# zitongbai/bipedal_control

Measured on AMD Instinct MI355X. Metric: MPC solves/s (H1, horizon=100), higher is better.
Workload: dtype f64; 1 GPU; Unitree H1 trot (template tiled from t = 0), horizon=100 intervals (dt 0.015), batch=256 per GPU perturbed initial states, cold start, 1 SQP iteration (BASELINE.json configs[1]); solver=sqp, global_batch=256, problems_on_rank0=256, shooting_nodes=108, nx=22, nu=22

## Files before the change

bipedal_control_amd/csrc/k_node.hip:

```cpp
#include <hip/hip_runtime.h>
#include <hip/hip_ext.h>

#include <stdexcept>

#include "kernel_launchers.h"
#include "launch.h"
#include "kernels/rollout.h"

namespace bpmpc {

template <int NJ>
__global__ __launch_bounds__(kWave) void k_prepare(Launch L) {
  constexpr int NX = 12 + NJ, NU = 12 + NJ;
  const int s = blockIdx.x, b = s / L.N, k = s % L.N;
  const int g = L.buf.p_grid[b];
  const int n = L.buf.g_nodes[g];
  if (k >= n) { if (threadIdx.x == 0) L.buf.n_info[s] = 0; return; }
  const size_t gs = (size_t)g * L.N + k;
  if (threadIdx.x == 0) L.buf.n_info[s] = 8 | ((L.buf.g_mode[gs] & 3) << 1) | (L.buf.g_kind[gs] == 1 ? 1 : 0);
  if (threadIdx.x < kNodeAux) {
    const int t = threadIdx.x;
    L.buf.n_aux[(size_t)s * kNodeAux + t] = t == 0 ? L.buf.g_dt[gs] : t < 5 ? L.buf.g_zref[gs * 4 + t - 1] : t < 9 ? L.buf.g_zdref[gs * 4 + t - 5] : 0.0;
  }
  prepare_node<NJ>(*L.model, L.buf.g_kind[gs], L.buf.g_mode[gs], L.buf.g_start[gs], L.cold != 0, k == n - 1, L.buf.p_tgt_n[b],
// ... 198 lines not shown
  constexpr int NX = 12 + NJ, NU = 12 + NJ, LPN = C::LPN, NPW = C::NPW;
  __shared__ LinFastNodeLds<NJ, false, CHAIN> lds[kTrialWaves * NPW];
  __shared__ LinFastShared<NJ, false> shared;
  const int sub = threadIdx.x / LPN, g = threadIdx.x % LPN;
  const int widx = blockIdx.x * (kTrialWaves * NPW) + sub;
  {
    const int total = L.batch * L.klen, w0 = blockIdx.x * (kTrialWaves * NPW), w1 = (w0 + kTrialWaves * NPW < total ? w0 + kTrialWaves * NPW : total) - 1;
    bool any = false;
    for (int pb = w0 / L.klen; pb <= w1 / L.klen; ++pb) any = any || L.buf.done[pb] == 0;
    if (!any) return;
  }
  bool valid = widx < L.batch * L.klen;
  const int b = valid ? widx / L.klen : 0, k = valid ? L.k0 + widx % L.klen : 0;
  const double* dx = L.buf.dx + ((size_t)b * (L.N + 1) + k) * NX;
  {
    const int fin = L.buf.done[b];
    const double alpha = L.buf.alpha[b];
    const int info = L.buf.n_info[(size_t)b * L.N + k];
    const size_t s0 = (size_t)b * L.N + k;
    const double* xk = L.buf.x + ((size_t)b * (L.N + 1) + k) * NX;
    const TrialPre pre = trial_preload<C>(xk, xk + NX, L.buf.u + s0 * NU, L.buf.xref + s0 * NX, dx, dx + NX, L.buf.du + s0 * NU, g, L.buf.n_aux + s0 * kNodeAux);
    load_shared_model<kTrialWaves * kWave>(*L.model, shared, threadIdx.x);
    NodeInputs in;
    in.kind = info & 1; in.mode = (info >> 1) & 3; in.dt = 0.0;
    in.x = xk; in.xnext = xk + NX; in.u = L.buf.u + s0 * NU; in.xref = L.buf.xref + s0 * NX; in.zref = nullptr; in.zdref = nullptr;
    __syncthreads();
    valid = valid && fin == 0 && info != 0;
    const size_t s = valid ? s0 : 0;
    trial_fast<NJ, C>(*L.model, shared, lds[sub], valid, in, alpha, dx, L.buf.du + s * NU, dx + NX, L.buf.trial_perf + s * 3, g, nullptr, &pre);
  }
}

template <int NJ, bool CHAIN>
__global__ __launch_bounds__(kTrialWaves * kWave) void k_constraint_values(Launch L, double* eqv) {
  using C = LinFastCfg<NJ, true, CHAIN>;
  constexpr int NX = 12 + NJ, NU = 12 + NJ, LPN = C::LPN, NPW = C::NPW;
  __shared__ LinFastNodeLds<NJ, false, CHAIN> lds[kTrialWaves * NPW];
  __shared__ LinFastShared<NJ, false> shared;
  load_shared_model<kTrialWaves * kWave>(*L.model, shared, threadIdx.x);
  __syncthreads();
  const int sub = threadIdx.x / LPN, g = threadIdx.x % LPN;
  const int widx = blockIdx.x * (kTrialWaves * NPW) + sub;
  bool valid = widx < L.batch * L.klen;
  const int b = valid ? widx / L.klen : 0, k = valid ? L.k0 + widx % L.klen : 0;
  const int grid = L.buf.p_grid[b];
  valid = valid && k < L.buf.g_nodes[grid] && L.buf.g_kind[(size_t)grid * L.N + k] == 0;
  const size_t s = valid ? (size_t)b * L.N + k : 0;
  const NodeInputs in = node_inputs<NJ>(L, b, k);
  const double* dx = L.buf.dx + ((size_t)b * (L.N + 1) + k) * NX;
  double perf[3];
  trial_fast<NJ, C, true>(*L.model, shared, lds[sub], valid, in, 0.0, dx, L.buf.du + s * NU, dx + NX, perf, g, eqv + s * kMaxEqRows);
}

template <int NJ, bool CHAIN>
__global__ __launch_bounds__(kWave) void k_rollout(const DeviceModel* model, RolloutArgs a) {
  __shared__ RolloutLds<NJ, CHAIN> w;
  load_shared_model<kWave>(*model, w.shared, threadIdx.x);
  __syncthreads();
  rollout_policy<NJ, CHAIN>(*model, w, a);
}

constexpr int kDecideThreads = 256;
template <int NJ>
__global__ __launch_bounds__(kDecideThreads) void k_ls_decide(Launch L, int look_first) {
  __shared__ double partial[3 * kDecideThreads + 5];
  linesearch_decide<NJ, kDecideThreads>(partial, problem_ls<NJ>(L, blockIdx.x), L.ls, look_first != 0);
// ... 75 lines not shown
      if (ev_start && ev_stop) hipExtLaunchKernelGGL(kernel, grid, block, 0, st, ev_start, ev_stop, 0, L);
      else hipLaunchKernelGGL(kernel, grid, block, 0, st, L);
    };
    if (L.ilqr) {
      if (!L.serial_legs) throw std::runtime_error("linearize_fast: the ILQR lineariser is instantiated for serial-leg robots only");
      if (materialise) launch(k_linearize_fast<NJ, true, true, true>);
      else launch(k_linearize_fast<NJ, false, true, true>);
    } else if (L.serial_legs) {
      if (materialise) launch(k_linearize_fast<NJ, true, true>);
      else launch(k_linearize_fast<NJ, false, true>);
    } else {
      if (materialise) launch(k_linearize_fast<NJ, true, false>);
      else launch(k_linearize_fast<NJ, false, false>);
    }
  });
}
void warm_shift(int nj, int slots, hipStream_t st, const Launch& L, const int* restarted) {
  KL_NJ(nj, hipLaunchKernelGGL(k_warm_shift<NJ>, dim3(slots), dim3(kWave), 0, st, L, restarted));
}
void ls_begin(int nj, int batch, hipStream_t st, const Launch& L) { KL_NJ(nj, hipLaunchKernelGGL(k_ls_begin<NJ>, dim3(batch), dim3(kWave), 0, st, L)); }
void trial_reference(int nj, int slots, hipStream_t st, const Launch& L) { KL_NJ(nj, hipLaunchKernelGGL(k_trial<NJ>, dim3(slots), dim3(kWave), 0, st, L)); }
int trial_fast_workgroups(int nj, int nodes) {
  const int per_wg = kTrialWaves * (nj == 10 ? LinFastCfg<10, true>::NPW : LinFastCfg<12, true>::NPW);
  return (nodes + per_wg - 1) / per_wg;
}
void trial_fast(int nj, int nodes, hipStream_t st, const Launch& L) {
  const int grid = trial_fast_workgroups(nj, nodes);
  KL_NJ(nj, {
    if (L.serial_legs) hipLaunchKernelGGL((k_trial_fast<NJ, true>), dim3(grid), dim3(kTrialWaves * kWave), 0, st, L);
    else hipLaunchKernelGGL((k_trial_fast<NJ, false>), dim3(grid), dim3(kTrialWaves * kWave), 0, st, L);
  });
}
void ls_decide(int nj, int batch, hipStream_t st, const Launch& L, bool look_first) { KL_NJ(nj, hipLaunchKernelGGL(k_ls_decide<NJ>, dim3(batch), dim3(kDecideThreads), 0, st, L, look_first ? 1 : 0)); }
void ls_tail(int nj, int batch, hipStream_t st, const Launch& L, int first_round, int max_trials, bool pending) {
  KL_NJ(nj, {
    if (L.serial_legs) hipLaunchKernelGGL((k_ls_tail<NJ, true>), dim3(batch), dim3(kTailThreads), 0, st, L, first_round, max_trials, pending ? 1 : 0);
    else hipLaunchKernelGGL((k_ls_tail<NJ, false>), dim3(batch), dim3(kTailThreads), 0, st, L, first_round, max_trials, pending ? 1 : 0);
  });
}
void constraint_values(int nj, int nodes, hipStream_t st, const Launch& L, double* eqv) {
  const int grid = trial_fast_workgroups(nj, nodes);
  KL_NJ(nj, {
    if (L.serial_legs) hipLaunchKernelGGL((k_constraint_values<NJ, true>), dim3(grid), dim3(kTrialWaves * kWave), 0, st, L, eqv);
    else hipLaunchKernelGGL((k_constraint_values<NJ, false>), dim3(grid), dim3(kTrialWaves * kWave), 0, st, L, eqv);
  });
}
void rollout(int nj, bool serial_legs, int batch, hipStream_t st, const DeviceModel* model, const RolloutArgs& a) {
  KL_NJ(nj, {
    constexpr bool kChainFits = LinFastCfg<NJ, false, true>::LPN == 16;
    const dim3 grid((batch + LinFastCfg<NJ>::NPW - 1) / LinFastCfg<NJ>::NPW);
    if constexpr (kChainFits) {
      if (serial_legs) { hipLaunchKernelGGL((k_rollout<NJ, true>), grid, dim3(kWave), 0, st, model, a); return; }
    }
    hipLaunchKernelGGL((k_rollout<NJ, false>), grid, dim3(kWave), 0, st, model, a);
  });
}
void copy_pairs(int grid, hipStream_t st, const double* a_src, double* a_dst, size_t na, const double* b_src, double* b_dst, size_t nb,
                int* iterations, int* active, int batch) {
  hipLaunchKernelGGL(k_copy_pairs, dim3(grid > 0 ? grid : 1), dim3(256), 0, st, a_src, a_dst, na, b_src, b_dst, nb, iterations, active, batch);
}

}
}
```

bipedal_control_amd/csrc/kernel_launchers.h:

```cpp
#pragma once
#include <hip/hip_runtime.h>

#include <cstddef>
#include <stdexcept>

namespace bpmpc {

#define KL_NJ(nj, ...)                                                          \
  do {                                                                          \
    if ((nj) == 10) { constexpr int NJ = 10; __VA_ARGS__; }                     \
    else if ((nj) == 12) { constexpr int NJ = 12; __VA_ARGS__; }                \
    else throw std::runtime_error("unsupported joint count");                   \
  } while (0)

struct Launch;
struct DeviceModel;
struct RolloutArgs;
struct DdpBuffers;
struct TickArgs;
struct RestartArgs;

namespace kl {

void prepare(int nj, int slots, hipStream_t st, const Launch& L);
void linearize_reference(int nj, int slots, hipStream_t st, const Launch& L);
void linearize_fast(int nj, bool materialise, int nodes, hipStream_t st, const Launch& L, hipEvent_t ev_start = nullptr, hipEvent_t ev_stop = nullptr);
void warm_shift(int nj, int slots, hipStream_t st, const Launch& L, const int* restarted = nullptr);
void ls_begin(int nj, int batch, hipStream_t st, const Launch& L);
void trial_reference(int nj, int slots, hipStream_t st, const Launch& L);
int trial_fast_workgroups(int nj, int nodes);
void trial_fast(int nj, int nodes, hipStream_t st, const Launch& L);
void ls_decide(int nj, int batch, hipStream_t st, const Launch& L, bool look_first = false);
void ls_tail(int nj, int batch, hipStream_t st, const Launch& L, int first_round, int max_trials, bool pending);
void constraint_values(int nj, int nodes, hipStream_t st, const Launch& L, double* eqv);
void rollout(int nj, bool serial_legs, int batch, hipStream_t st, const DeviceModel* model, const RolloutArgs& a);
void copy_pairs(int grid, hipStream_t st, const double* a_src, double* a_dst, size_t na, const double* b_src, double* b_dst, size_t nb,
                int* iterations, int* active, int batch);

void project_reference(int nj, int slots, hipStream_t st, const Launch& L);
void project_lu_s(int nj, int max_vel_rows, bool packed, int nodes, hipStream_t st, const Launch& L);
void project_fast(int nj, bool packed, bool joint_rows, int nodes, hipStream_t st, const Launch& L);

void riccati_reference(int nj, int batch, hipStream_t st, const Launch& L);
void riccati_fast(int nj, bool joint_rows, int batch, hipStream_t st, const Launch& L);
void riccati_fast8(int nj, bool joint_rows, int batch, hipStream_t st, const Launch& L);

void riccati_wave(int nj, bool two_per_simd, bool joint_rows, int batch, hipStream_t st, const Launch& L);
void riccati_rollout(int nj, int batch, hipStream_t st, const Launch& L);

void ddp_policy(int nj, int batch, hipStream_t st, const Launch& L, const DdpBuffers& d);
void ddp_cost(int nj, int batch, bool fast, hipStream_t st, const Launch& L, const DdpBuffers& d);
void ddp_select(int nj, int batch, hipStream_t st, const Launch& L, const DdpBuffers& d, double armijo);
void ddp_nominal(int nj, int batch, hipStream_t st, const Launch& L, const DdpBuffers& d);
void ddp_finish(int nj, int batch, hipStream_t st, const Launch& L, const DdpBuffers& d);
void ddp_keep_times(int batch, int N, hipStream_t st, const DdpBuffers& d, double* tp_time, int* tp_kind, int* tp_nodes, int* tp_grid);

void tick_observe_policy(int nj, int batch, hipStream_t st, const DeviceModel* model, const TickArgs& a);
void tick_commands(int nj, int batch, hipStream_t st, const double* x_opt, const double* u_opt, const double* sol, double* cmd);
void restart_observe(int nj, int batch, hipStream_t st, const DeviceModel* model, const RestartArgs& a);

}
}
```

bipedal_control_amd/csrc/kernels/linesearch.h:

```cpp
#pragma once
#include "node_lq.h"

namespace bpmpc {

constexpr int kMaxTargetPoints = 8;
constexpr int kStatsStride = 16;

struct LineSearchSettings {
  double g_max, g_min, alpha_decay, alpha_min, gamma_c, armijo_factor, delta_tol, cost_tol;
  int max_iterations;
};

template <int NJ>
BP_DEVICE void prepare_node(const DeviceModel& md, int kind, int mode, double t_start, bool cold, bool last, int n_pts, const double* tgt_t,
                            const double* tgt_x, const double* x0, double* xref, double* x, double* u, double* x_terminal) {
  constexpr int NX = 12 + NJ, NU = 12 + NJ;
  BP_LANES(tid, kWave) {
    if (tid < NX) {
      double val;
      if (n_pts == 1 || t_start <= tgt_t[0]) {
        val = tgt_x[tid];
      } else if (t_start >= tgt_t[n_pts - 1]) {
        val = tgt_x[(n_pts - 1) * NX + tid];
      } else {
// ... 170 lines not shown
#if defined(BPMPC_HOST_EMULATION)
        p.remaining[0] -= 1;
#else
        atomicSub(p.remaining, 1);
#endif
      } else {
        p.alpha[0] = next_alpha;
      }
    }
  }
  BP_SYNC();
  const bool accepted = partial[3 * NL] != 0.0;
  if (accepted) {
#if !defined(BPMPC_HOST_EMULATION)
#pragma unroll
    for (int j = 0; j < UPD; ++j) {
      const int idx = (int)threadIdx.x + j * NL;
      if (idx < nxe) p.x[idx] = xv[j] + alpha * dxv[j];
      if (idx < nue) p.u[idx] = uv[j] + alpha * duv[j];
    }
    int t0 = (int)threadIdx.x;
    if constexpr (!PRE) asm volatile("" : "+v"(t0));
    for (int idx = t0 + UPD * NL; idx < nxe; idx += NL) p.x[idx] += alpha * p.dx[idx];
    for (int idx = t0 + UPD * NL; idx < nue; idx += NL) p.u[idx] += alpha * p.du[idx];
#else
    BP_LANES(tid, NL) {
      for (int idx = tid; idx < (p.n_nodes + 1) * NX; idx += NL) p.x[idx] += alpha * p.dx[idx];
      for (int idx = tid; idx < p.n_nodes * NU; idx += NL) p.u[idx] += alpha * p.du[idx];
    }
#endif
  }
}

}
```

bipedal_control_amd/csrc/launch.h:

```cpp
#pragma once
#include <hip/hip_runtime.h>

#include <cstddef>

#include "device_model.h"
#include "kernels/linesearch.h"
#include "kernels/node_lq.h"
#include "kernels/project_node.h"
#include "kernels/riccati_fast.h"
#include "kernels/linearize_fast.h"

namespace bpmpc {

struct Buffers {
  int *g_kind, *g_mode, *g_nodes;
  double *g_dt, *g_start, *g_zref, *g_zdref;
  int* p_grid;
  double *p_x0, *p_tgt_t, *p_tgt_x;
  int* p_tgt_n;
  double *x, *u, *x_init, *u_init, *xref;
  double *A, *B, *b, *Q, *R, *P, *q, *r, *c, *C, *D, *e, *perf;
  int* nc;
  double *Px, *Pu, *Pe, *At, *Bt, *bt, *Qt, *Rt, *Pt, *qt, *rt;
  double *Wt, *Qp, *Mt;
  double* Vt;
  int* nut;
  int* n_info;
  double* n_aux;
  double* lin_park;
  double* lin_dump;
  double* qrd;
  double *Kt, *kt, *dx, *du, *K, *summary, *dx0;
  double *Acl, *bcl, *kff, *mvec, *mscal, *rprof;
  double *x_prev, *u_prev, *K_prev, *tp_time;
  int *tp_kind, *tp_nodes, *tp_grid;
  double *roll_t, *roll_x0, *roll_x, *roll_u;
  int *roll_steps, *roll_status;
  double *g_time, *rg_t0, *rg_start, *p_t0, *p_cmd, *lib_d;
  int *rg_gait, *rg_status, *rg_rows, *lib_i;
  double* ric_carry;
  double* zero_page;
  double *trial_perf, *base, *alpha, *stats;
  int *done, *active, *iterations, *remaining;
};

struct DdpBuffers {
  int cap;
  int nv;
  double alpha_v[kMaxDdpSteps];
  double* lff;
  double *rec_t, *rec_x, *rec_u, *cost;
  int* rec_n;
  double *end_x, *end_u;
  int *roll_steps, *roll_status;
  double *sol_t, *sol_x, *sol_u;
  int* sol_n;
  double *merit0, *merit, *alpha, *update_is;
  int *accepted, *failed, *n_points;
};

constexpr int kLinMaxEvents = 8;
struct Launch {
  const DeviceModel* model;
  Buffers buf;
  int batch, N;
  int k0, klen;
  int cold;
  int feedback;
  int serial_legs;
  LineSearchSettings ls;
  double reg_prim;
  int lin_ev_n, lin_inter;
  int lin_ev[kLinMaxEvents];
  int ilqr;
  double ilqr_shift;
};
// ... 41 lines not shown
  const size_t s0 = (size_t)b * L.N;
  p.n_nodes = L.buf.g_nodes[L.buf.p_grid[b]];
  p.node_perf = L.buf.perf + s0 * 3;
  p.trial_perf = L.buf.trial_perf + s0 * 3;
  p.x0 = L.buf.p_x0 + (size_t)b * NX;
  p.x = L.buf.x + (size_t)b * (L.N + 1) * NX;
  p.u = L.buf.u + s0 * NU;
  p.dx = L.buf.dx + (size_t)b * (L.N + 1) * NX;
  p.du = L.buf.du + s0 * NU;
  p.summary = L.buf.summary + (size_t)b * 4;
  p.base = L.buf.base + (size_t)b * 3;
  p.alpha = L.buf.alpha + b;
  p.done = L.buf.done + b;
  p.active = L.buf.active + b;
  p.iterations = L.buf.iterations + b;
  p.stats = L.buf.stats + (size_t)b * kStatsStride;
  p.remaining = L.buf.remaining;
  return p;
}

template <int NJ>
__device__ __forceinline__ bool riccati_fast_io(const Launch& L, RiccatiFastIO& io, double* lds_scratch ) {
  constexpr int NX = 12 + NJ, NU = 12 + NJ;
  const int b = blockIdx.x;
  const int tid_ = threadIdx.x;
  io.with_ls = L.k0 == 0;
  if (io.with_ls) io.ls = problem_ls<NJ>(L, b);
  if (!L.buf.active[b]) {
    if (io.with_ls && tid_ < kWave) linesearch_begin_wave<NJ>(lds_scratch, io.ls, tid_);
    return false;
  }
  const size_t s0 = (size_t)b * L.N;
  double* dx0 = L.buf.dx0 + (size_t)b * NX;
  if (tid_ < NX) dx0[tid_] = L.buf.p_x0[(size_t)b * NX + tid_] - L.buf.x[(size_t)b * (L.N + 1) * NX + tid_];
  __syncthreads();
  io.base.N = L.buf.g_nodes[L.buf.p_grid[b]];
  io.base.nut = L.buf.nut + s0;
  io.base.At = L.buf.At + s0 * NX * NX; io.base.Bt = L.buf.Bt + s0 * NX * NU; io.base.bt = L.buf.bt + s0 * NX;
  io.base.Qt = L.buf.Qt + s0 * NX * NX; io.base.Rt = L.buf.Rt + s0 * NU * NU; io.base.Pt = L.buf.Pt + s0 * NU * NX;
  io.base.qt = L.buf.qt + s0 * NX; io.base.rt = L.buf.rt + s0 * NU;
  io.Wt = L.buf.Wt + s0 * PackedLq<NJ>::W_SIZE; io.Qp = L.buf.Qp + s0 * PackedLq<NJ>::Q_SIZE; io.Mt = L.buf.Mt + s0 * PackedLq<NJ>::M_SIZE;
  io.base.Px = L.buf.Px + s0 * NU * NX; io.base.Pu = L.buf.Pu + s0 * NU * NU; io.base.Pe = L.buf.Pe + s0 * NU;
  io.Vt = L.buf.Vt + s0 * NJ * PackedLq<NJ>::WP;
  io.mode = L.buf.g_mode + (size_t)L.buf.p_grid[b] * L.N;
  io.zero_one = L.buf.zero_page;
  io.lqA = L.buf.A + s0 * NX * NX; io.lqB = L.buf.B + s0 * NX * NU; io.lqb = L.buf.b + s0 * NX; io.lqq = L.buf.q + s0 * NX; io.lqr = L.buf.r + s0 * NU;
  io.qrd = L.buf.qrd + s0 * kQrdStride; io.gdt = L.buf.g_dt + (size_t)L.buf.p_grid[b] * L.N;
  io.model = L.model;
  io.base.dx0 = dx0;
  io.base.Kt = nullptr; io.base.kt = nullptr;
  io.base.dx = L.buf.dx + (size_t)b * (L.N + 1) * NX; io.base.du = L.buf.du + s0 * NU;
  io.base.K = nullptr;
  io.base.summary = L.buf.summary + (size_t)b * 4;
  io.Acl = L.buf.Acl + s0 * NX * NX; io.bcl = L.buf.bcl + s0 * NX; io.kff = L.buf.kff + s0 * NU;
  io.mvec = L.buf.mvec + s0 * NX; io.mscal = L.buf.mscal + s0;
  io.Kfull = L.buf.K + s0 * NU * NX;
  io.prof = L.buf.rprof ? L.buf.rprof + (size_t)b * 8 : nullptr;
  io.k_lo = L.k0;
  io.k_hi = L.k0 + L.klen;
  io.carry = L.buf.ric_carry + (size_t)b * (NX * NX + NX + 2);
  io.reg = L.reg_prim;
  return true;
}

}
```

bipedal_control_amd/csrc/solver.h:

```cpp
#pragma once
#include <hip/hip_runtime.h>

#include <algorithm>
#include <cstring>
#include <map>
#include <string>
#include <utility>
#include <vector>

#include "../../include/bpmpc.h"
#include "capi_internal.h"
#include "device_model.h"
#include "kernel_launchers.h"
#include "launch.h"
#include "kernels/reference_device.h"

namespace bpmpc {

struct KernelTimer {
  std::vector<std::pair<hipEvent_t, hipEvent_t>> pending;
  double total_ms = 0.0;
  int launches = 0;
};

// ... 19 lines not shown
    used = 0; demand = 0;
  }
  void* take(size_t bytes) {
    const size_t at = (used + 63) & ~size_t(63);
    demand = ((demand + 63) & ~size_t(63)) + bytes;
    if (!base || at + bytes > cap) return nullptr;
    used = at + bytes;
    return base + at;
  }
  void release() { if (base) (void)hipHostFree(base); base = nullptr; cap = used = demand = 0; }
};

struct bpmpc_solver {
  HostStaging staging;
  PinnedArena pin_up, pin_down;
  char* xfer = nullptr;
  size_t xfer_cap = 0;
  RobotModel rm;
  DeviceModel dm;
  DeviceModel* d_model = nullptr;
  bpmpc_settings settings{};
  int nx = 0, nu = 0;
  int batch = 0, n_grids = 0, n_nodes_max = 0;
  int num_cus = 256;
  bool structured_project = false;
  int riccati_wave = 1;
  bool lin_compact = true;
  bool force_tables = false;
  bool wt_joint_rows = false;
  bool sweep_wave_regime() const { return riccati_wave == 2 || riccati_wave == 4 || ((riccati_wave == 1 || riccati_wave == 3) && batch > 2 * num_cus); }
  bool sweep_two_per_simd() const { return sweep_wave_regime() && (riccati_wave >= 3 || (riccati_wave == 1 && batch > 4 * num_cus)); }
  bool sweep_completes_joint_rows() const { return !wt_joint_rows && structured_project && !settings.reference_kernels; }
  int r8_rounds = 0;
  int eight_wave_rounds() const { return r8_rounds > 0 ? r8_rounds : (rm.nj == 10 ? 3 : 1); }
  bool sweep_eight_waves() const { return riccati_wave != 2 && riccati_wave != 4 && batch <= eight_wave_rounds() * num_cus; }
  bool has_solution = false;
  bool has_rollout = false;
  bool rollout_unchecked = false;
  double* tick_x = nullptr;
  bool loop_from_tick = false;
  int* restart_flag = nullptr;
  int* restart_mask = nullptr;
  double* restart_x = nullptr;
  bool restart_pending = false, restart_wait = false;
  std::vector<int> grid_kind;
  int max_rows = kMaxEqRows;
  int max_vel_rows = 12;
  bool cold = true;
  hipStream_t stream = nullptr;
  bool own_stream = false;
  hipStream_t producer_stream = nullptr;
  hipEvent_t ev_go = nullptr;
  std::vector<hipEvent_t> ev_chunk;
  Buffers buf{};
  std::vector<void*> allocations;
  std::map<std::string, std::pair<void*, size_t>> named;
  std::map<std::string, bool> is_int;
  std::vector<double> node_times;
  std::vector<int> grid_nodes, grid_of_problem;
  std::map<std::string, KernelTimer> timers;
  int* h_remaining = nullptr;
  LineSearchSettings ls{};

  template <typename T>
  T* alloc(const char* name, size_t count, bool integer = false) {
    void* p = nullptr;
// ... 152 lines not shown
```

bipedal_control_amd/csrc/solver.hip:

```cpp
#include <hip/hip_runtime.h>

#include <cmath>
#include <cstdint>
#include <algorithm>
#include <cstring>
#include <map>
#include <tuple>
#include <memory>
#include <stdexcept>
#include <string>
#include <vector>

#include "solver.h"
#include "reference_gen.h"
#include "kernels/rollout.h"

#define TIMED_ON(on, cls, ...)                                                      \
  do {                                                                              \
    hipEvent_t ev_a_, ev_b_;                                                        \
    time_begin(cls, &ev_a_, &ev_b_, on);                                            \
    __VA_ARGS__;                                                                    \
    time_end(cls, ev_a_, ev_b_, on);                                                \
    HIP_CHECK(hipGetLastError());                                                   \
  } while (0)
// ... 27 lines not shown
}
void bpmpc_solver::launch_project(hipStream_t on, const Launch& L, int nodes) {
  TIMED_ON(on, "project_lu", kl::project_lu_s(nj(), max_vel_rows, structured_project, nodes, on, L));
  TIMED_ON(on, "project", kl::project_fast(nj(), structured_project, !sweep_completes_joint_rows(), nodes, on, L));
}
void bpmpc_solver::stage_project() {
  const Launch L = launch_params();
  if (settings.reference_kernels) TIMED("project", kl::project_reference(nj(), batch * settings.max_nodes, stream, L));
  else launch_project(stream, L, batch * L.klen);
}
void bpmpc_solver::launch_riccati(const Launch& L) {
  if (sweep_eight_waves()) { TIMED("riccati", kl::riccati_fast8(nj(), !sweep_completes_joint_rows(), batch, stream, L)); return; }
  if (!sweep_wave_regime()) {
    TIMED("riccati", kl::riccati_fast(nj(), !sweep_completes_joint_rows(), batch, stream, L));
    return;
  }
  TIMED("riccati", { kl::riccati_wave(nj(), sweep_two_per_simd(), !sweep_completes_joint_rows(), batch, stream, L); if (L.k0 == 0) kl::riccati_rollout(nj(), batch, stream, L); });
}
void bpmpc_solver::stage_riccati() {
  const Launch L = launch_params();
  if (settings.reference_kernels) TIMED("riccati", kl::riccati_reference(nj(), batch, stream, L));
  else launch_riccati(L);
}
void bpmpc_solver::stage_linesearch() {
  const Launch L = launch_params();
  if (settings.reference_kernels) HIP_CHECK(hipMemsetAsync(buf.remaining, 0, sizeof(int), stream));
  hipEvent_t ev_a, ev_b;
  time_begin("linesearch", &ev_a, &ev_b);
  if (settings.reference_kernels) kl::ls_begin(nj(), batch, stream, L);
  int max_trials = 0;
  for (double a = 1.0; a >= ls.alpha_min; a *= ls.alpha_decay) ++max_trials;
  if (!settings.reference_kernels) {
    const int nodes = batch * L.klen;
    static const int wide_rounds = [] { const char* e = std::getenv("BPMPC_LS_WIDE_ROUNDS"); const int v = e ? std::atoi(e) : 2; return v < 1 ? 1 : v; }();
    int round = 0;
    bool pending = false;
    for (; round < wide_rounds && round < max_trials; ++round) {
      kl::trial_fast(nj(), nodes, stream, L);
      pending = round > 0 && (round + 1 == wide_rounds || round + 1 == max_trials);
      if (!pending) kl::ls_decide(nj(), batch, stream, L, round > 0);
    }
    kl::ls_tail(nj(), batch, stream, L, round, max_trials, pending);
    HIP_CHECK(hipGetLastError());
    time_end("linesearch", ev_a, ev_b);
    return;
  }
  for (int t = 0; t < max_trials; ++t) {
    kl::trial_reference(nj(), batch * settings.max_nodes, stream, L);
    kl::ls_decide(nj(), batch, stream, L);
    HIP_CHECK(hipGetLastError());
    HIP_CHECK(hipMemcpyAsync(h_remaining, buf.remaining, sizeof(int), hipMemcpyDeviceToHost, stream));
    HIP_CHECK(hipStreamSynchronize(stream));
    if (*h_remaining <= 0) break;
  }
  time_end("linesearch", ev_a, ev_b);
}
void bpmpc_solver::pipelined_backward() {
  const int chunks = settings.pipeline_chunks;
  const int n = n_nodes_max;
  HIP_CHECK(hipEventRecord(ev_go, stream));
  HIP_CHECK(hipStreamWaitEvent(producer_stream, ev_go, 0));
  for (int c = 0; c < chunks; ++c) {
    const int hi = n - (int)((long long)n * c / chunks), lo = n - (int)((long long)n * (c + 1) / chunks);
    if (hi <= lo) continue;
    Launch L = launch_params();
    L.k0 = lo;
    L.klen = hi - lo;
// ... 94 lines not shown
  b.x = s->alloc<double>("x", B * (N + 1) * NX); b.u = s->alloc<double>("u", S * NU);
  b.x_init = s->alloc<double>("x_init", B * (N + 1) * NX); b.u_init = s->alloc<double>("u_init", S * NU);
  b.xref = s->alloc<double>("xref", S * NX);
  b.A = s->alloc<double>("A", S * NX * NX); b.B = s->alloc<double>("B", S * NX * NU); b.b = s->alloc<double>("b", S * NX);
  b.Q = s->alloc<double>("Q", S * NX * NX); b.R = s->alloc<double>("R", S * NU * NU); b.P = s->alloc<double>("P", S * NU * NX);
  b.q = s->alloc<double>("q", S * NX); b.r = s->alloc<double>("r", S * NU); b.c = s->alloc<double>("c", S);
  b.C = s->alloc<double>("C", S * kMaxEqRows * NX); b.D = s->alloc<double>("D", S * kMaxEqRows * NU); b.e = s->alloc<double>("e", S * kMaxEqRows);
  b.perf = s->alloc<double>("perf", S * 3); b.nc = s->alloc<int>("nc", S, true);
  b.Px = s->alloc<double>("Px", S * NU * NX); b.Pu = s->alloc<double>("Pu", S * NU * NU); b.Pe = s->alloc<double>("Pe", S * NU);
  b.nut = s->alloc<int>("nut", S, true);
  b.n_info = s->alloc<int>("n_info", S, true);
  b.n_aux = s->alloc<double>("n_aux", S * kNodeAux);
  b.At = b.Bt = b.bt = b.Qt = b.Rt = b.Pt = b.qt = b.rt = b.Kt = b.kt = b.Wt = b.Qp = b.Mt = b.Vt = nullptr;
  if (s->settings.reference_kernels) {
    b.At = s->alloc<double>("At", S * NX * NX); b.Bt = s->alloc<double>("Bt", S * NX * NU); b.bt = s->alloc<double>("bt", S * NX);
    b.Qt = s->alloc<double>("Qt", S * NX * NX); b.Rt = s->alloc<double>("Rt", S * NU * NU); b.Pt = s->alloc<double>("Pt", S * NU * NX);
    b.qt = s->alloc<double>("qt", S * NX); b.rt = s->alloc<double>("rt", S * NU);
    b.Kt = s->alloc<double>("Kt", S * NU * NX); b.kt = s->alloc<double>("kt", S * NU);
  } else {
    const size_t wp = ((NX + 1 + NU + 15) / 16) * 16;
    b.Wt = s->alloc<double>("Wt", S * NX * wp); b.Qp = s->alloc<double>("Qp", S * NX * 32); b.Mt = s->alloc<double>("Mt", S * NU * wp);
    b.Vt = s->alloc<double>("Vt", S * (NX - 12) * wp);
  }
  b.dx = s->alloc<double>("dx", B * (N + 1) * NX); b.du = s->alloc<double>("du", S * NU);
  b.K = s->alloc<double>("K", S * NU * NX);
  b.Acl = s->alloc<double>("Acl", S * NX * NX); b.bcl = s->alloc<double>(nullptr, S * NX); b.kff = s->alloc<double>(nullptr, S * NU);
  b.mvec = s->alloc<double>(nullptr, S * NX); b.mscal = s->alloc<double>(nullptr, S);
  b.rprof = s->alloc<double>("rprof", std::max<size_t>(B * 8, 32768));
  b.summary = s->alloc<double>("summary", B * 4); b.dx0 = s->alloc<double>(nullptr, B * NX);
  b.trial_perf = s->alloc<double>("trial_perf", S * 3); b.base = s->alloc<double>("base", B * 3); b.alpha = s->alloc<double>("alpha", B);
  b.stats = s->alloc<double>("stats", B * kStatsStride);
  b.done = s->alloc<int>("done", B, true); b.active = s->alloc<int>("active", B, true); b.iterations = s->alloc<int>("iterations", B, true);
  b.remaining = s->alloc<int>(nullptr, 1);
  {
    const size_t tick = B * (64 + NX * 8 + N * 4 + (N + 1) * 8 + 64) + (size_t)kRefLibCapacity * 16 + 4096;
    const size_t solution = (B * ((N + 1) * NX + N * NU + N * NU * NX + kStatsStride)) * sizeof(double) + 4096;
    s->xfer_cap = std::max(tick, std::min<size_t>(size_t(1) << 20, solution));
    s->xfer = s->alloc<char>(nullptr, s->xfer_cap);
  }
  if (s->is_ddp()) {
    DdpBuffers& d = s->ddp;
    d.cap = (int)N + 1;
    {
      constexpr double kContractionRate = 0.5;
      d.nv = 0; d.alpha_v[d.nv++] = 0.0;
      for (double al = s->rm.ddp.ls_max_step_length; al >= s->rm.ddp.ls_min_step_length && d.nv < kMaxDdpSteps; al *= kContractionRate) d.alpha_v[d.nv++] = al;
    }
    const size_t P = B * (size_t)d.cap, V = (size_t)d.nv;
    d.lff = s->alloc<double>("ddp_lff", S * NU);
    d.rec_t = s->alloc<double>(nullptr, V * P); d.rec_x = s->alloc<double>(nullptr, V * P * NX); d.rec_u = s->alloc<double>(nullptr, V * P * NU); d.rec_n = s->alloc<int>("ddp_rec_n", V * B, true);
    d.cost = s->alloc<double>(nullptr, V * P * 3);
    d.end_x = s->alloc<double>(nullptr, V * B * NX); d.end_u = s->alloc<double>(nullptr, V * B * NU); d.roll_steps = s->alloc<int>("ddp_roll_steps", V * B * 2, true); d.roll_status = s->alloc<int>("ddp_roll_status", V * B, true);
    d.sol_t = s->alloc<double>("ddp_t", P); d.sol_x = s->alloc<double>(nullptr, P * NX); d.sol_u = s->alloc<double>("ddp_u", P * NU); d.sol_n = s->alloc<int>(nullptr, B);
    d.merit0 = s->alloc<double>(nullptr, B); d.merit = s->alloc<double>(nullptr, B); d.alpha = s->alloc<double>(nullptr, B);
    d.update_is = s->alloc<double>("ddp_update_is", B);
    d.accepted = s->alloc<int>(nullptr, B); d.failed = s->alloc<int>(nullptr, B); d.n_points = s->alloc<int>("ddp_points", B, true);
  }
}

template <typename T>
void upload(bpmpc_solver* s, T* dst, const std::vector<T>& src) {
  if (!src.empty()) HIP_CHECK(hipMemcpyAsync(dst, src.data(), src.size() * sizeof(T), hipMemcpyHostToDevice, s->stream));
}

void copy_pairs(bpmpc_solver* s, const double* a_src, double* a_dst, size_t na, const double* b_src, double* b_dst, size_t nb, bool rearm) {
  const size_t work = (na > nb ? na : nb) / 2;
// ... 497 lines not shown
    set_last_error("bpmpc_solver_create: no usable HIP device (this engine has no CPU path)");
    return BPMPC_ERR_NO_DEVICE;
  }
  std::unique_ptr<bpmpc_solver> s(new bpmpc_solver);
  const int rc = guarded(BPMPC_ERR_IO, [&]() -> int {
    s->rm = model_of(model);
    if (s->rm.nj != 10 && s->rm.nj != 12) { set_last_error("only 10- and 12-joint bipeds are instantiated"); return BPMPC_ERR_UNSUPPORTED; }
    if (settings->reg_prim != 0.0 && settings->reference_kernels) { set_last_error("reg_prim is implemented by the fast kernels only"); return BPMPC_ERR_UNSUPPORTED; }
    if (!(settings->reg_prim >= 0.0)) { set_last_error("reg_prim must be >= 0"); return BPMPC_ERR_INVALID_ARGUMENT; }
    s->dm = make_device_model(s->rm);
    s->settings = *settings;
    if (settings->solver != BPMPC_SOLVER_SQP && settings->solver != BPMPC_SOLVER_DDP) { set_last_error("bpmpc_solver_create: unknown solver"); return BPMPC_ERR_INVALID_ARGUMENT; }
    if (settings->feedback_policy < 0 || settings->feedback_policy > 2) { set_last_error("bpmpc_solver_create: feedback_policy must be 0, 1 or 2"); return BPMPC_ERR_INVALID_ARGUMENT; }
    if (settings->solver == BPMPC_SOLVER_DDP) {
      const DdpConfig& d = s->rm.ddp;
      if (d.algorithm != 1) { set_last_error("DDP: only ddp.algorithm ILQR is implemented (SLQ integrates continuous-time Riccati equations)"); return BPMPC_ERR_UNSUPPORTED; }
      if (d.strategy != 0) { set_last_error("DDP: only ddp.strategy LINE_SEARCH is implemented"); return BPMPC_ERR_UNSUPPORTED; }
      if (d.ls_hessian_correction_strategy != 0) { set_last_error("DDP: only lineSearch.hessianCorrectionStrategy DIAGONAL_SHIFT is implemented"); return BPMPC_ERR_UNSUPPORTED; }
      if (d.max_num_iterations != 1 || settings->sqp_iterations > 1) { set_last_error("DDP: one ILQR iteration per run (ddp.maxNumIterations 1): later iterations live on the roll-out's adaptive time grid"); return BPMPC_ERR_UNSUPPORTED; }
      if (!(d.ls_min_step_length > 0.0) || !(d.ls_max_step_length >= d.ls_min_step_length)) { set_last_error("DDP: lineSearch.minStepLength / maxStepLength"); return BPMPC_ERR_INVALID_ARGUMENT; }
      if (d.use_feedback_policy && settings->feedback_policy != 2) { set_last_error("DDP: ddp.useFeedbackPolicy true is not implemented (the gains live on the nominal grid, the solution on the roll-out's time points)"); return BPMPC_ERR_UNSUPPORTED; }
      if (settings->feedback_policy == 1) { set_last_error("DDP: feedback_policy 1 (LinearController) is not implemented for the DDP solution"); return BPMPC_ERR_UNSUPPORTED; }
      s->settings.return_gains = 1;
      s->settings.pipeline_chunks = 1;
    }
    s->nx = s->rm.nx; s->nu = s->rm.nu;
    HIP_CHECK(hipSetDevice(settings->device));
    { hipDeviceProp_t prop; HIP_CHECK(hipGetDeviceProperties(&prop, settings->device)); s->num_cus = prop.multiProcessorCount; }
    { const char* e = std::getenv("BPMPC_WT_JOINT_ROWS"); s->wt_joint_rows = e && e[0] == '1'; }
    { const char* e = std::getenv("BPMPC_LIN_TABLES"); s->force_tables = e && e[0] == '1'; }
    { const char* e = std::getenv("BPMPC_LIN_COMPACT"); s->lin_compact = !(e && e[0] == '0'); }
    { const char* e = std::getenv("BPMPC_RICCATI_WAVE"); s->riccati_wave = e ? std::atoi(e) : 1; }
    { const char* e = std::getenv("BPMPC_R8_ROUNDS"); s->r8_rounds = e ? std::atoi(e) : 0; }
    {
      bool block_diagonal = true;
      for (int c = 0; c < 12; ++c)
        for (int j = 12; j < s->nu; ++j) block_diagonal = block_diagonal && s->dm.R[c * s->nu + j] == 0.0 && s->dm.R[j * s->nu + c] == 0.0;
      const char* e = std::getenv("BPMPC_DENSE_PROJECT");
      s->structured_project = block_diagonal && !(e && e[0] == '1');
    }
    if (s->is_ddp() && !(s->dm.serial_legs && !s->force_tables)) s->settings.reference_kernels = 1;
    if (settings->stream) { s->stream = static_cast<hipStream_t>(settings->stream); }
    else { HIP_CHECK(hipStreamCreateWithFlags(&s->stream, hipStreamNonBlocking)); s->own_stream = true; }
    if (s->settings.pipeline_chunks <= 0) s->settings.pipeline_chunks = 1;
    if (s->settings.pipeline_chunks > 16) s->settings.pipeline_chunks = 16;
    HIP_CHECK(hipStreamCreateWithFlags(&s->producer_stream, hipStreamNonBlocking));
    HIP_CHECK(hipEventCreateWithFlags(&s->ev_go, hipEventDisableTiming));
    s->ev_chunk.resize(s->settings.pipeline_chunks);
    for (auto& e : s->ev_chunk) HIP_CHECK(hipEventCreateWithFlags(&e, hipEventDisableTiming));
    {
      std::vector<char> host(kLinImageOffset + sizeof(LinFastShared<12, true>), 0);
      std::memcpy(host.data(), &s->dm, sizeof(DeviceModel));
      if (s->rm.nj == 10) fill_shared_image<10>(s->dm, *reinterpret_cast<LinFastShared<10, true>*>(host.data() + kLinImageOffset));
      else if (s->rm.nj == 12) fill_shared_image<12>(s->dm, *reinterpret_cast<LinFastShared<12, true>*>(host.data() + kLinImageOffset));
      HIP_CHECK(hipMalloc(reinterpret_cast<void**>(&s->d_model), host.size()));
      HIP_CHECK(hipMemcpy(s->d_model, host.data(), host.size(), hipMemcpyHostToDevice));
    }
    HIP_CHECK(hipHostMalloc(reinterpret_cast<void**>(&s->h_remaining), sizeof(int)));
    const SqpConfig& q = s->rm.sqp;
    s->ls = LineSearchSettings{q.g_max, q.g_min, q.alpha_decay, q.alpha_min, q.gamma_c, q.armijo_factor, q.delta_tol, q.cost_tol,
                               settings->sqp_iterations > 0 ? settings->sqp_iterations : q.sqp_iteration};
    allocate(s.get());
    HIP_CHECK(hipStreamSynchronize(s->stream));
    return BPMPC_OK;
  });
  if (rc != BPMPC_OK) { bpmpc_solver_destroy(s.release()); return rc; }
// ... 200 lines not shown
```

Baseline: 342,000 solves/s.

## Fuse line-search decision and next trial into one split-per-problem kernel

Adds a k_ls_step kernel in which each workgroup of a problem redundantly reduces the previous trial's merit sums, decides acceptance, applies its share of the accepted step update, and then evaluates the next trial at the decayed alpha. Done, alpha and trial-performance buffers are double-buffered between rounds. This replaces the separate decide and trial launches of the wide rounds when the grid is small relative to CU count, which removes a launch and a global round trip per line-search round. In exchange every workgroup repeats the reduction, and the kernel is pinned to a waves-per-EU hint.

```diff
diff --git a/bipedal_control_amd/csrc/k_node.hip b/bipedal_control_amd/csrc/k_node.hip
--- a/bipedal_control_amd/csrc/k_node.hip
+++ b/bipedal_control_amd/csrc/k_node.hip
@@ -254,6 +254,41 @@
 }
 
 template <int NJ, bool CHAIN>
+__global__ __launch_bounds__(kTrialWaves * kWave) __attribute__((amdgpu_waves_per_eu(3, 3)))
+void k_ls_step(Launch L, int S, int* done_next, double* alpha_next, double* trial_perf_next) {
+  using C = LinFastCfg<NJ, true, CHAIN>;
+  constexpr int NX = 12 + NJ, NU = 12 + NJ, LPN = C::LPN, NPW = C::NPW, NL = kTrialWaves * kWave;
+  __shared__ LinFastNodeLds<NJ, false, CHAIN> lds[kTrialWaves * NPW];
+  __shared__ LinFastShared<NJ, false> shared;
+  static_assert(sizeof(lds) >= (3 * NL + 5) * sizeof(double), "the decision's sums fit the node storage");
+  double* partial = reinterpret_cast<double*>(&lds[0]);
+  const int b = blockIdx.x / S, s = blockIdx.x - b * S;
+  if (L.buf.done[b]) {
+    if (s == 0 && threadIdx.x == 0) { done_next[b] = 1; alpha_next[b] = L.buf.alpha[b]; }
+    return;
+  }
+  double alpha;
+  if (!linesearch_step_decide<NJ, NL>(partial, problem_ls<NJ>(L, b), L.ls, L.buf.ls_xfirst + (size_t)b * NX, s, S, done_next + b, alpha_next + b, alpha)) return;
+  const int sub = threadIdx.x / LPN, g = threadIdx.x % LPN;
+  const int slot = s * (kTrialWaves * NPW) + sub;
+  bool valid = slot < L.klen;
+  const int k = valid ? L.k0 + slot : 0;
+  const size_t s0 = (size_t)b * L.N + k;
+  const int info = L.buf.n_info[s0];
+  const double* xk = L.buf.x + ((size_t)b * (L.N + 1) + k) * NX;
+  const double* dx = L.buf.dx + ((size_t)b * (L.N + 1) + k) * NX;
+  const TrialPre pre = trial_preload<C>(xk, xk + NX, L.buf.u + s0 * NU, L.buf.xref + s0 * NX, dx, dx + NX, L.buf.du + s0 * NU, g, L.buf.n_aux + s0 * kNodeAux);
+  load_shared_model<NL>(*L.model, shared, threadIdx.x);
+  NodeInputs in;
+  in.kind = info & 1; in.mode = (info >> 1) & 3; in.dt = 0.0;
+  in.x = xk; in.xnext = xk + NX; in.u = L.buf.u + s0 * NU; in.xref = L.buf.xref + s0 * NX; in.zref = nullptr; in.zdref = nullptr;
+  __syncthreads();
+  valid = valid && info != 0;
+  const size_t sv = valid ? s0 : 0;
+  trial_fast<NJ, C>(*L.model, shared, lds[sub], valid, in, alpha, dx, L.buf.du + sv * NU, dx + NX, trial_perf_next + sv * 3, g, nullptr, &pre);
+}
+
+template <int NJ, bool CHAIN>
 __global__ __launch_bounds__(kTrialWaves * kWave) void k_constraint_values(Launch L, double* eqv) {
   using C = LinFastCfg<NJ, true, CHAIN>;
   constexpr int NX = 12 + NJ, NU = 12 + NJ, LPN = C::LPN, NPW = C::NPW;
@@ -395,6 +430,13 @@
   });
 }
 void ls_decide(int nj, int batch, hipStream_t st, const Launch& L, bool look_first) { KL_NJ(nj, hipLaunchKernelGGL(k_ls_decide<NJ>, dim3(batch), dim3(kDecideThreads), 0, st, L, look_first ? 1 : 0)); }
+void ls_step(int nj, int batch, hipStream_t st, const Launch& L, int* done_next, double* alpha_next, double* trial_perf_next) {
+  const int S = trial_fast_workgroups(nj, L.klen);
+  KL_NJ(nj, {
+    if (L.serial_legs) hipLaunchKernelGGL((k_ls_step<NJ, true>), dim3(batch * S), dim3(kTrialWaves * kWave), 0, st, L, S, done_next, alpha_next, trial_perf_next);
+    else hipLaunchKernelGGL((k_ls_step<NJ, false>), dim3(batch * S), dim3(kTrialWaves * kWave), 0, st, L, S, done_next, alpha_next, trial_perf_next);
+  });
+}
 void ls_tail(int nj, int batch, hipStream_t st, const Launch& L, int first_round, int max_trials, bool pending) {
   KL_NJ(nj, {
     if (L.serial_legs) hipLaunchKernelGGL((k_ls_tail<NJ, true>), dim3(batch), dim3(kTailThreads), 0, st, L, first_round, max_trials, pending ? 1 : 0);
diff --git a/bipedal_control_amd/csrc/kernel_launchers.h b/bipedal_control_amd/csrc/kernel_launchers.h
--- a/bipedal_control_amd/csrc/kernel_launchers.h
+++ b/bipedal_control_amd/csrc/kernel_launchers.h
@@ -31,6 +31,7 @@
 int trial_fast_workgroups(int nj, int nodes);
 void trial_fast(int nj, int nodes, hipStream_t st, const Launch& L);
 void ls_decide(int nj, int batch, hipStream_t st, const Launch& L, bool look_first = false);
+void ls_step(int nj, int batch, hipStream_t st, const Launch& L, int* done_next, double* alpha_next, double* trial_perf_next);
 void ls_tail(int nj, int batch, hipStream_t st, const Launch& L, int first_round, int max_trials, bool pending);
 void constraint_values(int nj, int nodes, hipStream_t st, const Launch& L, double* eqv);
 void rollout(int nj, bool serial_legs, int batch, hipStream_t st, const DeviceModel* model, const RolloutArgs& a);
diff --git a/bipedal_control_amd/csrc/kernels/linesearch.h b/bipedal_control_amd/csrc/kernels/linesearch.h
--- a/bipedal_control_amd/csrc/kernels/linesearch.h
+++ b/bipedal_control_amd/csrc/kernels/linesearch.h
@@ -226,4 +226,113 @@
   }
 }
 
-}
+#if !defined(BPMPC_HOST_EMULATION)
+template <int NJ, int NL>
+__device__ __forceinline__ bool linesearch_step_decide(double* partial , const ProblemLS& p, const LineSearchSettings& st,
+                                                       const double* x_first, int share, int shares, int* done_next, double* alpha_next, double& alpha_out) {
+  constexpr int NX = 12 + NJ, NU = 12 + NJ;
+  static_assert(NL == 256, "the sums are those of linesearch_decide<NJ, 256>: its first 256 lanes");
+  constexpr int UPD = 2;
+  const int nxe = (p.n_nodes + 1) * NX, nue = p.n_nodes * NU;
+  const int first = share * NL + (int)threadIdx.x, stride = shares * NL;
+  double xv[UPD], dxv[UPD], uv[UPD], duv[UPD];
+#pragma unroll
+  for (int j = 0; j < UPD; ++j) {
+    const int idx = first + j * stride;
+    const int ix = idx < nxe ? idx : 0, iu = idx < nue ? idx : 0;
+    xv[j] = p.x[ix]; dxv[j] = p.dx[ix]; uv[j] = p.u[iu]; duv[j] = p.du[iu];
+  }
+  const double alpha = p.alpha[0];
+  const int tid = (int)threadIdx.x;
+  {
+    double a = 0.0, b = 0.0, c = 0.0;
+    for (int k = tid; k < p.n_nodes; k += NL) { a += p.trial_perf[3 * k]; b += p.trial_perf[3 * k + 1]; c += p.trial_perf[3 * k + 2]; }
+    if (tid < NX) { const double d = p.x0[tid] - (x_first[tid] + alpha * p.dx[tid]); b += d * d; }
+    partial[tid] = a; partial[NL + tid] = b; partial[2 * NL + tid] = c;
+  }
+  __syncthreads();
+  if (tid < 3) {
+    int lim = p.n_nodes > NX ? p.n_nodes : NX;
+    if (lim > NL) lim = NL;
+    double s = 0.0;
+    const double* row = partial + tid * NL;
+    int i = 0;
+    for (; i + 8 <= lim; i += 8) {
+      double v[8];
+#pragma unroll
+      for (int j = 0; j < 8; ++j) v[j] = row[i + j];
+#pragma unroll
+      for (int j = 0; j < 8; ++j) s += v[j];
+    }
+    for (; i < lim; ++i) s += row[i];
+    partial[3 * NL + 2 + tid] = s;
+  }
+  __syncthreads();
+  if (tid == 0) {
+    const double merit = partial[3 * NL + 2], dyn = partial[3 * NL + 3], eq = partial[3 * NL + 4];
+    const double merit0 = p.base[0];
+    const double viol0 = sqrt(p.base[1] + p.base[2]);
+    const double viol = sqrt(dyn + eq);
+    const double descent = alpha * p.summary[0];
+    bool accepted;
+    if (viol > st.g_max) {
+      accepted = viol < (1.0 - st.gamma_c) * viol0;
+    } else if (viol < st.g_min && viol0 < st.g_min && descent < 0.0) {
+      accepted = merit < merit0 + st.armijo_factor * descent;
+    } else {
+      accepted = merit < (merit0 - st.gamma_c * viol0) || viol < (1.0 - st.gamma_c) * viol0;
+    }
+    const bool numerical = p.summary[3] != 0.0;
+    if (numerical) accepted = false;
+    const double next_alpha = alpha * st.alpha_decay;
+    const bool tiny = next_alpha * sqrt(p.summary[1]) < st.delta_tol && next_alpha * sqrt(p.summary[2]) < st.delta_tol;
+    const bool give_up = !accepted && (numerical || tiny || !(next_alpha >= st.alpha_min));
+    partial[3 * NL] = accepted ? 1.0 : 0.0;
+    partial[3 * NL + 1] = give_up ? 1.0 : 0.0;
+    partial[3 * NL + 2] = next_alpha;
+    if (share == 0) {
+      if (accepted || give_up) {
+        double* s = p.stats;
+        const int it = p.iterations[0] + 1;
+        p.iterations[0] = it;
+        const double dxn = accepted ? alpha * sqrt(p.summary[1]) : 0.0, dun = accepted ? alpha * sqrt(p.summary[2]) : 0.0;
+        s[0] = (double)p.n_nodes;
+        s[1] = (double)it;
+        s[2] = numerical ? 2.0 : (accepted ? 0.0 : 1.0);
+        s[3] = merit0; s[4] = p.base[1]; s[5] = p.base[2];
+        s[6] = accepted ? merit : merit0; s[7] = accepted ? dyn : p.base[1]; s[8] = accepted ? eq : p.base[2];
+        s[9] = accepted ? alpha : 0.0;
+        s[10] = p.summary[0];
+        s[11] = dxn; s[12] = dun;
+        bool keep_going = it < st.max_iterations;
+        if (keep_going && s[9] < st.alpha_min) keep_going = false;
+        if (keep_going && fabs(s[6] - merit0) < st.cost_tol && sqrt(s[7] + s[8]) < st.g_min) keep_going = false;
+        if (keep_going && dxn < st.delta_tol && dun < st.delta_tol) keep_going = false;
+        p.active[0] = keep_going ? 1 : 0;
+        done_next[0] = 1;
+        alpha_next[0] = alpha;
+        atomicSub(p.remaining, 1);
+      } else {
+        done_next[0] = 0;
+        alpha_next[0] = next_alpha;
+      }
+    }
+  }
+  __syncthreads();
+  const bool accepted = partial[3 * NL] != 0.0, give_up = partial[3 * NL + 1] != 0.0;
+  alpha_out = partial[3 * NL + 2];
+  if (accepted) {
+#pragma unroll
+    for (int j = 0; j < UPD; ++j) {
+      const int idx = first + j * stride;
+      if (idx < nxe) p.x[idx] = xv[j] + alpha * dxv[j];
+      if (idx < nue) p.u[idx] = uv[j] + alpha * duv[j];
+    }
+    for (int idx = first + UPD * stride; idx < nxe; idx += stride) p.x[idx] += alpha * p.dx[idx];
+    for (int idx = first + UPD * stride; idx < nue; idx += stride) p.u[idx] += alpha * p.du[idx];
+  }
+  return !(accepted || give_up);
+}
+#endif
+
+}
diff --git a/bipedal_control_amd/csrc/launch.h b/bipedal_control_amd/csrc/launch.h
--- a/bipedal_control_amd/csrc/launch.h
+++ b/bipedal_control_amd/csrc/launch.h
@@ -42,6 +42,8 @@
   double* zero_page;
   double *trial_perf, *base, *alpha, *stats;
   int *done, *active, *iterations, *remaining;
+  double *trial_perf_alt, *alpha_alt, *ls_xfirst;
+  int* done_alt;
 };
 
 struct DdpBuffers {
@@ -149,7 +151,11 @@
   }
   const size_t s0 = (size_t)b * L.N;
   double* dx0 = L.buf.dx0 + (size_t)b * NX;
-  if (tid_ < NX) dx0[tid_] = L.buf.p_x0[(size_t)b * NX + tid_] - L.buf.x[(size_t)b * (L.N + 1) * NX + tid_];
+  if (tid_ < NX) {
+    const double x_first = L.buf.x[(size_t)b * (L.N + 1) * NX + tid_];
+    dx0[tid_] = L.buf.p_x0[(size_t)b * NX + tid_] - x_first;
+    L.buf.ls_xfirst[(size_t)b * NX + tid_] = x_first;
+  }
   __syncthreads();
   io.base.N = L.buf.g_nodes[L.buf.p_grid[b]];
   io.base.nut = L.buf.nut + s0;
diff --git a/bipedal_control_amd/csrc/solver.h b/bipedal_control_amd/csrc/solver.h
--- a/bipedal_control_amd/csrc/solver.h
+++ b/bipedal_control_amd/csrc/solver.h
@@ -75,6 +75,8 @@
   bool sweep_two_per_simd() const { return sweep_wave_regime() && (riccati_wave >= 3 || (riccati_wave == 1 && batch > 4 * num_cus)); }
   bool sweep_completes_joint_rows() const { return !wt_joint_rows && structured_project && !settings.reference_kernels; }
   int r8_rounds = 0;
+  int ls_wide_rounds = 2;
+  bool ls_step = true;
   int eight_wave_rounds() const { return r8_rounds > 0 ? r8_rounds : (rm.nj == 10 ? 3 : 1); }
   bool sweep_eight_waves() const { return riccati_wave != 2 && riccati_wave != 4 && batch <= eight_wave_rounds() * num_cus; }
   bool has_solution = false;
diff --git a/bipedal_control_amd/csrc/solver.hip b/bipedal_control_amd/csrc/solver.hip
--- a/bipedal_control_amd/csrc/solver.hip
+++ b/bipedal_control_amd/csrc/solver.hip
@@ -83,7 +83,24 @@
   for (double a = 1.0; a >= ls.alpha_min; a *= ls.alpha_decay) ++max_trials;
   if (!settings.reference_kernels) {
     const int nodes = batch * L.klen;
-    static const int wide_rounds = [] { const char* e = std::getenv("BPMPC_LS_WIDE_ROUNDS"); const int v = e ? std::atoi(e) : 2; return v < 1 ? 1 : v; }();
+    const int wide_rounds = ls_wide_rounds;
+    if (ls_step && (long long)batch * kl::trial_fast_workgroups(nj(), L.klen) <= 8LL * num_cus) {
+      kl::trial_fast(nj(), nodes, stream, L);
+      Launch R = L;
+      int round = 1;
+      for (; round < wide_rounds && round < max_trials; ++round) {
+        const bool alt = R.buf.done == buf.done;
+        int* done_next = alt ? buf.done_alt : buf.done;
+        double* alpha_next = alt ? buf.alpha_alt : buf.alpha;
+        double* perf_next = alt ? buf.trial_perf_alt : buf.trial_perf;
+        kl::ls_step(nj(), batch, stream, R, done_next, alpha_next, perf_next);
+        R.buf.done = done_next; R.buf.alpha = alpha_next; R.buf.trial_perf = perf_next;
+      }
+      kl::ls_tail(nj(), batch, stream, R, round, max_trials, true);
+      HIP_CHECK(hipGetLastError());
+      time_end("linesearch", ev_a, ev_b);
+      return;
+    }
     int round = 0;
     bool pending = false;
     for (; round < wide_rounds && round < max_trials; ++round) {
@@ -244,6 +261,8 @@
   b.stats = s->alloc<double>("stats", B * kStatsStride);
   b.done = s->alloc<int>("done", B, true); b.active = s->alloc<int>("active", B, true); b.iterations = s->alloc<int>("iterations", B, true);
   b.remaining = s->alloc<int>(nullptr, 1);
+  b.trial_perf_alt = s->alloc<double>(nullptr, S * 3); b.alpha_alt = s->alloc<double>(nullptr, B); b.done_alt = s->alloc<int>(nullptr, B);
+  b.ls_xfirst = s->alloc<double>(nullptr, B * NX);
   {
     const size_t tick = B * (64 + NX * 8 + N * 4 + (N + 1) * 8 + 64) + (size_t)kRefLibCapacity * 16 + 4096;
     const size_t solution = (B * ((N + 1) * NX + N * NU + N * NU * NX + kStatsStride)) * sizeof(double) + 4096;
@@ -807,6 +826,8 @@
     { const char* e = std::getenv("BPMPC_LIN_COMPACT"); s->lin_compact = !(e && e[0] == '0'); }
     { const char* e = std::getenv("BPMPC_RICCATI_WAVE"); s->riccati_wave = e ? std::atoi(e) : 1; }
     { const char* e = std::getenv("BPMPC_R8_ROUNDS"); s->r8_rounds = e ? std::atoi(e) : 0; }
+    { const char* e = std::getenv("BPMPC_LS_WIDE_ROUNDS"); const int v = e ? std::atoi(e) : 2; s->ls_wide_rounds = v < 1 ? 1 : v; }
+    { const char* e = std::getenv("BPMPC_LS_STEP"); s->ls_step = !(e && e[0] == '0'); }
     {
       bool block_diagonal = true;
       for (int c = 0; c < 12; ++c)
```

Result: no change. 340,400 solves/s (-0.5%).
